# voithru/voice-activity-detection

Hardware: AMD Instinct MI355X
Metric: audio frames/sec (whole node) (higher is better)
Workload: dtype f32 (bf16x6 split operands, f32 accumulate)

## Files before the change

### __graft_entry__.py

```python
from __future__ import annotations

import sys
from pathlib import Path

REPO = Path(__file__).resolve().parent
if str(REPO) not in sys.path:
    sys.path.insert(0, str(REPO))


def build() -> None:
    from voice_activity_detection_amd import _lib, build as b

    so = b.build(force=True, verbose=True)
    b.build_variant(b.FAULT_LIB, b.FAULT_DEFINES, force=True, verbose=True)
    from oracle import oracle

    oracle.build(force=True)
    lib = _lib.load()
    import subprocess

    chk = subprocess.run([sys.executable, str(REPO / "scripts" / "check_async_loads.py"), "--lib", str(so)], capture_output=True, text=True)
    if chk.returncode != 0:
        raise RuntimeError("scripts/check_async_loads.py flags the built library:\n" + (chk.stdout + chk.stderr)[-3000:])
    import voice_activity_detection_amd as pkg

    assert pkg.SelfAttentiveVAD is not None
    print(f"built {so} [{lib.savad_version().decode()}] and {oracle.build()}")


def smoke() -> None:
    import numpy as np
    import torch

    from oracle import oracle
    from voice_activity_detection_amd import SelfAttentiveVAD, VADFromScratchPredictor, seeded_features, seeded_state_dict

    assert torch.cuda.is_available(), "smoke() needs a HIP device"
    state = seeded_state_dict(1234)
    model = SelfAttentiveVAD(80, 3, 128, 0.5)
    model.load_state_dict({k: torch.from_numpy(v) for k, v in state.items()})
    model = model.to("cuda:0").eval()
    worst = 0.0
    worst_s = 0.0
    for shape in ((8, 7, 80), (2, 96, 80)):
        x = seeded_features(7, shape)
        ref = oracle.forward(state, x)
        for prec, rm in (("fp32", 0), ("fp32s", 0)) + ((("fp32s", 7), ("fp32s", 8)) if shape[1] <= 32 else (("fp32s", 3),)):
            model.precision, model.row_mode = prec, rm
            try:
                with torch.no_grad():
                    y = model(features=torch.from_numpy(x).to("cuda:0")).cpu().numpy()
            finally:
                model.precision, model.row_mode = "fp32", 0
            err = float(np.abs(y - ref).max())
            if prec == "fp32":
                worst = max(worst, err)
            else:
                worst_s = max(worst_s, err)
            assert err < 1e-4, f"log-prob mismatch {err} at {shape} ({prec}, row_mode {rm})"
    feat = seeded_features(8, (120, 80))
    probs = VADFromScratchPredictor(model, "cuda:0").predict_probabilities(feat)
    ref_probs, _ = oracle.predict_probabilities(state, feat)
    perr = float(np.abs(probs - ref_probs).max())
    assert perr < 1e-4, perr
    x7 = seeded_features(9, (40, 7, 80))
    model.precision = "bf16"
    try:
        with torch.no_grad():
            y16 = model(features=torch.from_numpy(x7).to("cuda:0")).cpu().numpy()
    finally:
        model.precision = "fp32"
    e16 = float(np.abs(y16 - oracle.forward(state, x7)).max())
    assert e16 < 1.2e-2, f"bf16 log-prob mismatch {e16}"
    from oracle import logmel
    from voice_activity_detection_amd.features import log_mel

    audio = (np.random.default_rng(3).standard_normal(16000) * 0.1).astype(np.float32)
    emel = float(np.abs(log_mel(audio, "cuda:0").cpu().numpy() - logmel.log_mel(audio)).max())
    assert emel < 5e-4, f"log-mel mismatch {emel}"
    from oracle import resample as oresample
    from voice_activity_detection_amd.features import resample_to_16k_device

    clip = (np.random.default_rng(4).standard_normal(4000) * 0.1).astype(np.float32)
    assert np.array_equal(resample_to_16k_device(torch.from_numpy(clip).to("cuda:0"), 44100).cpu().numpy(), oresample.resample(clip, 44100)), "resampler bits"
    print(f"smoke ok: max |dlogp| = {worst:.2e} (fp32s: {worst_s:.2e}), predictor max |dp| = {perr:.2e}, bf16 T=7 max |dlogp| = {e16:.2e}, log-mel max |d| = {emel:.2e}")


if __name__ == "__main__":
    build()
    if "--smoke" in sys.argv:
        smoke()
```

### voice_activity_detection_amd/build.py

```python
from __future__ import annotations

import os
import shutil
import subprocess
import sys
from pathlib import Path

PKG = Path(__file__).resolve().parent
SRC = PKG / "csrc" / "savad.hip"
DEPS = (sorted((PKG / "csrc").glob("*.h")) + sorted((PKG / "csrc").glob("*.hip")) + sorted((PKG / "csrc").glob("*.inc")) +
        [PKG.parent / "include" / "savad.h"])
LIB = PKG / "libsavad.so"


def hipcc() -> str:
    for cand in (os.environ.get("HIPCC"), shutil.which("hipcc"), "/opt/rocm/bin/hipcc"):
        if cand and Path(cand).exists():
            return cand
    raise RuntimeError("hipcc not found (set HIPCC or install ROCm under /opt/rocm)")


def is_stale() -> bool:
    return not LIB.exists() or any(d.stat().st_mtime > LIB.stat().st_mtime for d in DEPS)


def build(force: bool = False, verbose: bool = False) -> Path:
    if not force and not is_stale():
        return LIB
    cmd = [hipcc(), "--offload-arch=gfx950", "-O3", "-std=c++17", "-shared", "-fPIC", "-fvisibility=hidden",
           "-Wno-unused-value", str(SRC), "-o", str(LIB)]
    if verbose:
        print(" ".join(cmd), file=sys.stderr)
    subprocess.run(cmd, check=True)
    return LIB


def build_variant(out: Path, defines=(), force: bool = False, verbose: bool = False) -> Path:
    out = Path(out)
    if not force and out.exists() and all(d.stat().st_mtime <= out.stat().st_mtime for d in DEPS):
        return out
    out.parent.mkdir(parents=True, exist_ok=True)
    cmd = [hipcc(), "--offload-arch=gfx950", "-O3", "-std=c++17", "-shared", "-fPIC", "-fvisibility=hidden", "-Wno-unused-value",
           *[f"-D{d}" for d in defines], str(SRC), "-o", str(out)]
    if verbose:
        print(" ".join(cmd), file=sys.stderr)
    subprocess.run(cmd, check=True)
    return out


FAULT_LIB = PKG.parent / "tests" / "fault" / "libsavad_fault17.so"
FAULT_DEFINES = ["SAVAD_FAULT_INJECT=17"]


if __name__ == "__main__":
    print(build(force="--force" in sys.argv, verbose=True))
```

### voice_activity_detection_amd/csrc/savad_device.h

```cpp
#pragma once
#include <hip/hip_runtime.h>
#include <stdint.h>

#include "savad_dims.h"

namespace savad {

constexpr int XLD = D + 4;
constexpr float LN_EPS = 1e-5f;
constexpr float NEG_BIG = -1.0e30f;
constexpr float RESCALE_LOG2 = 16.0f;

typedef float f32x2 __attribute__((ext_vector_type(2)));
typedef float f32x4 __attribute__((ext_vector_type(4)));
typedef float f32x16 __attribute__((ext_vector_type(16)));

#define SAVAD_MFMA(a, b, c) __builtin_amdgcn_mfma_f32_32x32x2f32((a), (b), (c), 0, 0, 0)

__device__ __forceinline__ f32x4 ld4(const float* p) { return *reinterpret_cast<const f32x4*>(p); }
__device__ __forceinline__ void st4(float* p, f32x4 v) { *reinterpret_cast<f32x4*>(p) = v; }
__device__ __forceinline__ void both_halves(float v, float& lo, float& hi) {
    const unsigned u = __builtin_bit_cast(unsigned, v);
    const auto r = __builtin_amdgcn_permlane32_swap(u, u, false, false);
    const unsigned a = r[0], b = r[1];
    lo = __builtin_bit_cast(float, a);
    hi = __builtin_bit_cast(float, b);
}
__device__ __forceinline__ float half_sum(float v) {
    float lo, hi;
    both_halves(v, lo, hi);
    return lo + hi;
}
__device__ __forceinline__ float half_max(float v) {
    float lo, hi;
    both_halves(v, lo, hi);
    return fmaxf(lo, hi);
}

__device__ __forceinline__ f32x16 zero16() {
    f32x16 z;
#pragma unroll
    for (int i = 0; i < 16; ++i) z[i] = 0.0f;
    return z;
}

__device__ __forceinline__ void add_bias(f32x16& acc, const float* __restrict__ b, int h) {
#pragma unroll
    for (int g = 0; g < 4; ++g) {
        const f32x4 b4 = ld4(b + 8 * g + 4 * h);
#pragma unroll
        for (int s = 0; s < 4; ++s) acc[4 * g + s] += b4[s];
    }
}

__device__ __forceinline__ size_t x_row_offset(size_t r, int T, int F, long xbs) {
    return xbs == (long)T * F ? r * (size_t)F : (r / (size_t)T) * (size_t)xbs + (r % (size_t)T) * (size_t)F;
}

__device__ __forceinline__ void store_block(float* rowp , const f32x16& v, int h) {
#pragma unroll
    for (int g = 0; g < 4; ++g) {
        f32x4 t;
#pragma unroll
        for (int s = 0; s < 4; ++s) t[s] = v[4 * g + s];
        st4(rowp + 8 * g + 4 * h, t);
    }
}
__device__ __forceinline__ void add_block(f32x16& v, const float* rowp, int h) {
#pragma unroll
    for (int g = 0; g < 4; ++g) {
        const f32x4 t = ld4(rowp + 8 * g + 4 * h);
#pragma unroll
        for (int s = 0; s < 4; ++s) v[4 * g + s] += t[s];
    }
}

__device__ __forceinline__ void layernorm_regs(const f32x16 (&x)[4], f32x4 (&xg)[16]) {
    float s = 0.0f;
#pragma unroll
    for (int nb = 0; nb < 4; ++nb)
#pragma unroll
        for (int r = 0; r < 16; ++r) s += x[nb][r];
    s = half_sum(s);
    const float mean = s * (1.0f / D);
    float ss = 0.0f;
#pragma unroll
    for (int nb = 0; nb < 4; ++nb)
#pragma unroll
        for (int r = 0; r < 16; ++r) {
            const float d = x[nb][r] - mean;
            xg[4 * nb + (r >> 2)][r & 3] = d;
            ss += d * d;
        }
    ss = half_sum(ss);
    const float rstd = 1.0f / sqrtf(ss * (1.0f / D) + LN_EPS);
#pragma unroll
    for (int G = 0; G < 16; ++G) xg[G] *= rstd;
}

__device__ __forceinline__ void wait_vmem_all() {
    __builtin_amdgcn_s_waitcnt(0x0F70);
    asm volatile("" ::: "memory");
}

__device__ __forceinline__ bool xcd_balanced_map(int B, int per_seq, int& b, int& rr) {
    const long W = (long)B * per_seq;
    const int per_xcd = (int)((W + 7) / 8);
    const int xcd = blockIdx.x & 7, slot = blockIdx.x >> 3;
    const long lin = (long)xcd * per_xcd + slot;
    if (slot >= per_xcd || lin >= W) return false;
    b = (int)(lin / per_seq);
    rr = (int)(lin % per_seq);
    return true;
}

#ifdef SAVAD_TIMING
__device__ long long g_savad_dbg[64];
#define SAVAD_STAMP(i)                                                                  \
    do {                                                                                \
        if (blockIdx.x == 0 && threadIdx.x == 0) g_savad_dbg[i] = __builtin_readcyclecounter(); \
    } while (0)
#else
#define SAVAD_STAMP(i) \
    do {               \
    } while (0)
#endif
#ifndef SAVAD_FAULT_INJECT
#define SAVAD_FAULT_INJECT 0
#endif
#ifndef SAVAD_ABLATE
#define SAVAD_ABLATE 0
#endif

__device__ __forceinline__ void stage_bias(float* dst, const float* __restrict__ src, int count) {
    for (int i = threadIdx.x * 4; i < count; i += 256 * 4) st4(dst + i, ld4(src + i));
}
struct BiasPiece {
    float* dst;
    const float* src;
    int count;
};
template <int N>
struct BiasRegs {
    f32x4 v[N];
};
template <int N>
__device__ __forceinline__ BiasRegs<N> request_bias_pieces(const BiasPiece (&p)[N]) {
    const int i = threadIdx.x * 4;
    BiasRegs<N> r;
#pragma unroll
    for (int n = 0; n < N; ++n) {
        const int j = i < p[n].count ? i : (p[n].count >= 4 ? p[n].count - 4 : 0);
        r.v[n] = ld4(p[n].src + j);
    }
    return r;
}
template <int N>
__device__ __forceinline__ void commit_bias_pieces(const BiasPiece (&p)[N], const BiasRegs<N>& r) {
    const int i = threadIdx.x * 4;
#pragma unroll
    for (int n = 0; n < N; ++n)
        if (i < p[n].count) st4(p[n].dst + i, r.v[n]);
}
template <int N>
__device__ __forceinline__ void stage_bias_pieces(const BiasPiece (&p)[N]) {
    commit_bias_pieces(p, request_bias_pieces(p));
}
__device__ __forceinline__ f32x16 bias_block(const float* lds_bias , int h) {
    f32x16 r;
#pragma unroll
    for (int g = 0; g < 4; ++g) {
        const f32x4 b4 = ld4(lds_bias + 8 * g + 4 * h);
#pragma unroll
        for (int e = 0; e < 4; ++e) r[4 * g + e] = b4[e];
    }
    return r;
}

struct WindowOffsets {
    int w;
    int off[64];
};


__device__ __forceinline__ constexpr int acc_row(int r, int h) { return 8 * (r >> 2) + 4 * h + (r & 3); }

__device__ __forceinline__ bool packed_key_ok(int B, int T, int blk, int m, int jk) {
    const int G = 32 / T;
    return (jk < G * T) && (jk / T == m / T) && (blk * G + jk / T < B);
}

__device__ __forceinline__ f32x2 classify_rows(const f32x4 (&xg)[16], const float* wc, const float* bc, int h) {
    float z0 = 0.0f, z1 = 0.0f;
#pragma unroll
    for (int G = 0; G < 16; ++G) {
        const f32x4 c0 = ld4(wc + 8 * G + 4 * h), c1 = ld4(wc + D + 8 * G + 4 * h);
#pragma unroll
        for (int e = 0; e < 4; ++e) {
            z0 = __builtin_fmaf(xg[G][e], c0[e], z0);
            z1 = __builtin_fmaf(xg[G][e], c1[e], z1);
        }
    }
    z0 = half_sum(z0) + bc[0];
    z1 = half_sum(z1) + bc[1];
    const float mx = fmaxf(z0, z1);
    const float lse = mx + logf(expf(z0 - mx) + expf(z1 - mx));
    return f32x2{z0 - lse, z1 - lse};
}

}
```

### voice_activity_detection_amd/csrc/savad_kernels_f32s.h

```cpp
#pragma once
#include "savad_kernels_bf16.h"
#include <type_traits>

namespace savad {
#ifdef SAVAD_TIMING
__device__ long long g_savad_wg[1024][4];
#endif
namespace fs {

using bf::bf16x8;
using bf::u32x4;
using bf::ldfrag;
using bf::stfrag;
using bf::FRAG_BYTES;
using bf::slot_row;
using bf::AttnState;
using bf::attn_state_init;
using bf::online_softmax_shifted;

constexpr int SLOT_BYTES = 2 * BLK3_BYTES;
constexpr int NRING3 = 3;
constexpr int ROW_LDS_BYTES = NRING3 * SLOT_BYTES + 9 * D * 4;

struct Tri {
    bf16x8 h, m, l;
};

__device__ __forceinline__ void split1(float a, __bf16& h, __bf16& m, __bf16& l) {
    h = (__bf16)a;
    if (SAVAD_ABLATE & 128) {
        m = l = h;
        return;
    }
    const float r1 = a - (float)h;
    m = (__bf16)r1;
    const float r2 = r1 - (float)m;
    l = (__bf16)r2;
}
__device__ __forceinline__ Tri split8(const float (&v)[8]) {
    Tri t;
#pragma unroll
    for (int e = 0; e < 8; ++e) {
        __bf16 h, m, l;
        split1(v[e], h, m, l);
        t.h[e] = h;
        t.m[e] = m;
        t.l[e] = l;
    }
    return t;
}
__device__ __forceinline__ Tri split_half(const f32x16& v, int j) {
    float t[8];
#pragma unroll
    for (int e = 0; e < 8; ++e) t[e] = v[8 * j + e];
    return split8(t);
}
__device__ __forceinline__ void split_row(const f32x4 (&xg)[16], Tri (&xp)[8]) {
#pragma unroll
    for (int ks = 0; ks < 8; ++ks) {
        float t[8];
#pragma unroll
        for (int e = 0; e < 8; ++e) t[e] = xg[2 * ks + (e >> 2)][e & 3];
        xp[ks] = split8(t);
    }
}
__device__ __forceinline__ Tri ldtri(const char* p ) {
    return Tri{ldfrag(p), ldfrag(p + FRAG_BYTES), ldfrag(p + 2 * FRAG_BYTES)};
}
__device__ __forceinline__ void sttri(char* p, const Tri& t) {
    stfrag(p, t.h);
    stfrag(p + FRAG_BYTES, t.m);
    stfrag(p + 2 * FRAG_BYTES, t.l);
}
__device__ __forceinline__ Tri zero_tri() {
    const bf16x8 z = __builtin_bit_cast(bf16x8, u32x4{0u, 0u, 0u, 0u});
    return Tri{z, z, z};
}

#define SAVAD_MF(a, b, c) __builtin_amdgcn_mfma_f32_32x32x16_bf16((a), (b), (c), 0, 0, 0)
template <bool SWAP>
__device__ __forceinline__ void mfma6x2_lo(f32x16& acc0, f32x16& acc1, const Tri& a0, const Tri& a1, const Tri& b) {
#define SAVAD_MF2(pa, pb)                                                           \
    acc0 = SWAP ? SAVAD_MF(b.pb, a0.pa, acc0) : SAVAD_MF(a0.pa, b.pb, acc0);        \
    acc1 = SWAP ? SAVAD_MF(b.pb, a1.pa, acc1) : SAVAD_MF(a1.pa, b.pb, acc1);
    SAVAD_MF2(h, l) SAVAD_MF2(l, h) SAVAD_MF2(m, m)
}
template <bool SWAP>
__device__ __forceinline__ void mfma6x2_hi(f32x16& acc0, f32x16& acc1, const Tri& a0, const Tri& a1, const Tri& b) {
    SAVAD_MF2(h, m) SAVAD_MF2(m, h) SAVAD_MF2(h, h)
#undef SAVAD_MF2
}
template <bool SWAP>
__device__ __forceinline__ void mfma6x2(f32x16& acc0, f32x16& acc1, const Tri& a0, const Tri& a1, const Tri& b) {
    mfma6x2_lo<SWAP>(acc0, acc1, a0, a1, b);
    mfma6x2_hi<SWAP>(acc0, acc1, a0, a1, b);
}

__device__ __forceinline__ void load_hblock32(f32x16 (&x)[4], const float* hb, int lane) {
#pragma unroll
    for (int nb = 0; nb < 4; ++nb)
#pragma unroll
        for (int g = 0; g < 4; ++g) {
            const f32x4 t = ld4(hb + ((nb * 4 + g) * 64 + lane) * 4);
#pragma unroll
            for (int s = 0; s < 4; ++s) x[nb][4 * g + s] += t[s];
        }
}
__device__ __forceinline__ void request_hblock32(f32x4 (&hr)[16], const float* hb , int lane) {
#define SAVAD_H_LD(i)                                                                                                          \
    asm volatile("global_load_dwordx4 %0, %1, %2 offset:%3" : "+v"(hr[i]) : "v"((unsigned)lane * 16u + 4096u * ((i) / 4)), "s"(hb), \
                 "n"(((i) % 4) * 1024) : "memory")
    SAVAD_H_LD(0); SAVAD_H_LD(1); SAVAD_H_LD(2); SAVAD_H_LD(3); SAVAD_H_LD(4); SAVAD_H_LD(5); SAVAD_H_LD(6); SAVAD_H_LD(7);
    SAVAD_H_LD(8); SAVAD_H_LD(9); SAVAD_H_LD(10); SAVAD_H_LD(11); SAVAD_H_LD(12); SAVAD_H_LD(13); SAVAD_H_LD(14); SAVAD_H_LD(15);
#undef SAVAD_H_LD
}
__device__ __forceinline__ void landed_hblock32(f32x4 (&hr)[16]) {
    asm volatile("" : "+v"(hr[0]), "+v"(hr[1]), "+v"(hr[2]), "+v"(hr[3]), "+v"(hr[4]), "+v"(hr[5]), "+v"(hr[6]), "+v"(hr[7]), "+v"(hr[8]),
                 "+v"(hr[9]), "+v"(hr[10]), "+v"(hr[11]), "+v"(hr[12]), "+v"(hr[13]), "+v"(hr[14]), "+v"(hr[15]));
}
__device__ __forceinline__ void store_hblock32(float* hb, const f32x16 (&x)[4], int lane) {
#pragma unroll
    for (int nb = 0; nb < 4; ++nb)
#pragma unroll
        for (int g = 0; g < 4; ++g) {
            f32x4 t;
#pragma unroll
            for (int s = 0; s < 4; ++s) t[s] = x[nb][4 * g + s];
            st4(hb + ((nb * 4 + g) * 64 + lane) * 4, t);
        }
}

#ifndef SAVAD_PIECE_FENCE
#define SAVAD_PIECE_FENCE 0x6
#endif
__device__ __forceinline__ const char* scalar_ptr(const char* p) {
    const size_t a = (size_t)p;
    const unsigned lo = __builtin_amdgcn_readfirstlane((unsigned)a), hi = __builtin_amdgcn_readfirstlane((unsigned)(a >> 32));
    return (const char*)((size_t)lo | ((size_t)hi << 32));
}
struct DmaJob {
    const char* src;
    unsigned ldsb;
};
struct Ring3 {
    static constexpr int PER = 12;
    char* base;
    int w, lane;
    unsigned voff[3];

    __device__ __forceinline__ Ring3(char* smem, int w_, int lane_) : base(smem), w(w_), lane(lane_) {
#pragma unroll
        for (int g = 0; g < 3; ++g) voff[g] = (unsigned)lane_ * 16u + 4096u * g;
    }
    __device__ __forceinline__ char* slot(int t) const { return base + (t % NRING3) * SLOT_BYTES; }
    __device__ __forceinline__ DmaJob job(int t, const char* seg0, const char* seg1) const {
        const unsigned slot0 = __builtin_amdgcn_readfirstlane((unsigned)(size_t)slot(t));
        return DmaJob{((w >> 1) ? seg1 : seg0) + (size_t)(w & 1) * (BLK3_BYTES / 2), slot0 + (unsigned)w * (BLK3_BYTES / 2)};
    }
    template <int I>
    __device__ __forceinline__ void piece(const DmaJob& j) const {
        if (SAVAD_ABLATE & 1) return;
        __builtin_amdgcn_sched_barrier(SAVAD_PIECE_FENCE);
        piece_raw<I>(j);
        __builtin_amdgcn_sched_barrier(SAVAD_PIECE_FENCE);
    }
    template <int I>
    __device__ __forceinline__ void piece_raw(const DmaJob& j) const {
        asm volatile(
            "s_add_u32 m0, %2, %3\n\t"
            "s_nop 0\n\t"
            "global_load_lds_dwordx4 %0, %1 offset:%4"
            :
            : "v"(voff[I / 4]), "s"(j.src), "s"(j.ldsb), "n"((I / 4) * 4096), "n"((I % 4) * 1024)
            : "memory", "scc");
    }
    __device__ __forceinline__ void issue_all(const DmaJob& j) const {
        if (SAVAD_ABLATE & 1) return;
        piece_raw<0>(j); piece_raw<1>(j); piece_raw<2>(j); piece_raw<3>(j); piece_raw<4>(j); piece_raw<5>(j);
        piece_raw<6>(j); piece_raw<7>(j); piece_raw<8>(j); piece_raw<9>(j); piece_raw<10>(j); piece_raw<11>(j);
    }
    template <int NEWER>
    __device__ __forceinline__ void acquire() const {
        if (SAVAD_ABLATE & 2) return;
        __builtin_amdgcn_s_waitcnt(bf::Ring<4>::vmcnt_imm(NEWER * PER));
        asm volatile("" ::: "memory");
        __syncthreads();
    }
};

struct NoMid {
    template <int KS>
    __device__ __forceinline__ void operator()(std::integral_constant<int, KS>) const {}
};
template <bool SWAP, bool DMA, class Mid = NoMid>
__device__ __forceinline__ void gemm_slot(f32x16& acc0, f32x16& acc1, const char* slot, const Tri (&xp)[8], const Ring3& ring,
                                          const DmaJob& job, const Mid& mid = Mid{}) {
    if (SAVAD_ABLATE & 8) {
#pragma unroll
        for (int ks = 0; ks < 8; ++ks) mfma6x2<SWAP>(acc0, acc1, xp[7 - ks], xp[ks ^ 1], xp[ks]);
        return;
    }
    const unsigned a = (unsigned)(size_t)slot + (unsigned)ring.lane * 16u;
    u32x4 f[2][6];
#define SAVAD_G_LD(ks, i) asm volatile("ds_read_b128 %0, %1 offset:%2" : "=v"(f[(ks) & 1][i]) : "v"(a), "n"(((i) / 3) * BLK3_BYTES + (ks) * TFRAG_BYTES + ((i) % 3) * FRAG_BYTES))
#define SAVAD_G_LD6(ks) SAVAD_G_LD(ks, 0); SAVAD_G_LD(ks, 1); SAVAD_G_LD(ks, 2); SAVAD_G_LD(ks, 3); SAVAD_G_LD(ks, 4); SAVAD_G_LD(ks, 5)
#define SAVAD_G_STEP(ks, P0, P1)                                                                                              \
    {                                                                                                                         \
        if constexpr ((ks) + 1 < 8) { SAVAD_G_LD6((ks) + 1); }                                                                \
        asm volatile("s_waitcnt lgkmcnt(%6)"                                                                                  \
                     : "+v"(f[(ks) & 1][0]), "+v"(f[(ks) & 1][1]), "+v"(f[(ks) & 1][2]), "+v"(f[(ks) & 1][3]), "+v"(f[(ks) & 1][4]), \
                       "+v"(f[(ks) & 1][5])                                                                                   \
                     : "n"((ks) + 1 < 8 ? 6 : 0));                                                                            \
        const Tri w0_{__builtin_bit_cast(bf16x8, f[(ks) & 1][0]), __builtin_bit_cast(bf16x8, f[(ks) & 1][1]),                  \
                      __builtin_bit_cast(bf16x8, f[(ks) & 1][2])};                                                            \
        const Tri w1_{__builtin_bit_cast(bf16x8, f[(ks) & 1][3]), __builtin_bit_cast(bf16x8, f[(ks) & 1][4]),                  \
                      __builtin_bit_cast(bf16x8, f[(ks) & 1][5])};                                                            \
        mfma6x2_lo<SWAP>(acc0, acc1, w0_, w1_, xp[ks]);                                                                       \
        if constexpr (DMA && (P1) >= 0) ring.template piece<((P1) >= 0 ? (P1) : 0)>(job);                                     \
        mid(std::integral_constant<int, (ks)>{});                                                                             \
        mfma6x2_hi<SWAP>(acc0, acc1, w0_, w1_, xp[ks]);                                                                       \
        if constexpr (DMA) ring.template piece<P0>(job);                                                                      \
    }
    SAVAD_G_LD6(0);
    SAVAD_G_STEP(0, 1, 0) SAVAD_G_STEP(1, 2, -1) SAVAD_G_STEP(2, 4, 3) SAVAD_G_STEP(3, 5, -1)
    SAVAD_G_STEP(4, 7, 6) SAVAD_G_STEP(5, 8, -1) SAVAD_G_STEP(6, 10, 9) SAVAD_G_STEP(7, 11, -1)
#undef SAVAD_G_STEP
#undef SAVAD_G_LD6
#undef SAVAD_G_LD
}

__global__ void pack_weight_frags3_kernel(const float* __restrict__ W, int N, int K, __bf16* __restrict__ out) {
    const int KS = K / 16;
    const size_t total = (size_t)(N / 32) * KS * 64 * 8;
    for (size_t i = (size_t)blockIdx.x * blockDim.x + threadIdx.x; i < total; i += (size_t)gridDim.x * blockDim.x) {
        const int e = (int)(i & 7);
        const int lane = (int)((i >> 3) & 63);
        const size_t f = i >> 9;
        const int ks = (int)(f % KS);
        const int nblk = (int)(f / KS);
        const int n = lane & 31, h = lane >> 5;
        const int k = 32 * (ks >> 1) + 16 * (ks & 1) + 8 * (e >> 2) + 4 * h + (e & 3);
        __bf16 ph, pm, pl;
        split1(W[(size_t)(32 * nblk + n) * K + k], ph, pm, pl);
        const size_t o = f * 3 * 512 + (size_t)lane * 8 + e;
        out[o] = ph;
        out[o + 512] = pm;
        out[o + 1024] = pl;
    }
}

__global__ void fold_vo_kernel(const float* __restrict__ Wo, const float* __restrict__ Wv, const float* __restrict__ bqkv,
                               float* __restrict__ Wvo, float* __restrict__ bvo) {
    const int n = blockIdx.x, k = threadIdx.x;
    double acc = 0.0, accb = 0.0;
    for (int j = 0; j < D; ++j) {
        const double w = (double)Wo[(size_t)n * D + j];
        acc += w * (double)Wv[(size_t)j * D + k];
        accb += w * (double)bqkv[2 * D + j];
    }
    Wvo[(size_t)n * D + k] = (float)acc;
    if (k == 0) bvo[n] = (float)accb;
}

__global__ void fold_qk_kernel(const float* __restrict__ Wq, const float* __restrict__ Wk, const float* __restrict__ bq, double c,
                               float* __restrict__ Wqt, float* __restrict__ bqt) {
    const int n = blockIdx.x, k = threadIdx.x;
    double acc = 0.0, accb = 0.0;
    for (int o = 0; o < D; ++o) {
        const double w = (double)Wk[(size_t)o * D + n];
        acc += w * (double)Wq[(size_t)o * D + k];
        accb += w * (double)bq[o];
    }
    Wqt[(size_t)n * D + k] = (float)(c * acc);
    if (k == 0) bqt[n] = (float)(c * accb);
}

template <int RB, int HALF, bool DMA, bool SCALE, class Mid = NoMid>
__device__ __forceinline__ void qkv_slot(const char* slot, const Tri (&xp)[8], const float* lb, char* __restrict__ dst, int blk,
                                         const Ring3& ring, const DmaJob& job, float qscale, bool live, const Mid& mid = Mid{}) {
    const int lane = ring.lane, n = lane & 31, h = lane >> 5;
    constexpr int nb0 = 2 * HALF;
    f32x16 acc[2];
    if constexpr (RB < 2) {
#pragma unroll
        for (int i = 0; i < 2; ++i) acc[i] = bias_block(lb + 32 * (nb0 + i), h);
        gemm_slot<false, DMA>(acc[0], acc[1], slot, xp, ring, job, mid);
    } else {
#pragma unroll
        for (int i = 0; i < 2; ++i) {
            const float bv = lb[32 * (nb0 + i) + n];
#pragma unroll
            for (int r = 0; r < 16; ++r) acc[i][r] = bv;
        }
        gemm_slot<true, DMA>(acc[0], acc[1], slot, xp, ring, job, mid);
    }
    if constexpr (SCALE) {
        acc[0] *= qscale;
        acc[1] *= qscale;
    }
    if (!live) return;
#pragma unroll
    for (int i = 0; i < 2; ++i)
#pragma unroll
        for (int j = 0; j < 2; ++j)
            sttri(dst + (size_t)blk * BLK3_BYTES + (2 * (nb0 + i) + j) * TFRAG_BYTES + lane * 16, split_half(acc[i], j));
}
template <int S, bool QKF, bool DMA, class Mid = NoMid>
__device__ __forceinline__ void qkv_image_slot(const char* slot, const Tri (&xp)[8], const float* lbq, char* __restrict__ qf, char* __restrict__ kf,
                                               char* __restrict__ vtf, int blk, const Ring3& ring, const DmaJob& job, float qscale, bool live,
                                               const Mid& mid = Mid{}) {
    constexpr int pos = S >> 1, rb = QKF ? 2 * pos : pos;
    qkv_slot<rb, (S & 1), DMA, (rb == 0 && !QKF)>(slot, xp, lbq + D * pos, rb == 0 ? qf : (rb == 1 ? kf : vtf), blk, ring, job, qscale, live, mid);
}

#ifndef SAVAD_KSTORE
#define SAVAD_KSTORE 2
#endif
__device__ __forceinline__ void store_k_tri(char* kblk , const Tri (&xp)[8], int ks, int lane) {
    sttri(kblk + ks * TFRAG_BYTES + lane * 16, xp[ks]);
}
__device__ __forceinline__ void store_k_burst(char* kblk, const Tri (&xp)[8], int lane, bool live) {
    if (!live) return;
#pragma unroll
    for (int ks = 0; ks < 8; ++ks) store_k_tri(kblk, xp, ks, lane);
}
template <int S>
struct KStoreMid {
    char* kblk;
    const Tri (&xp)[8];
    int lane;
    bool live;
    template <int KS>
    __device__ __forceinline__ void operator()(std::integral_constant<int, KS>) const {
        if constexpr ((KS & 1) && ((SAVAD_KSTORE == 2 && S == 0) || SAVAD_KSTORE == 3)) {
            __builtin_amdgcn_sched_barrier(SAVAD_PIECE_FENCE);
            if (live) {
                if constexpr (SAVAD_KSTORE == 2) {
                    store_k_tri(kblk, xp, KS - 1, lane);
                    store_k_tri(kblk, xp, KS, lane);
                } else {
                    store_k_tri(kblk, xp, 4 * S + (KS >> 1), lane);
                }
            }
            __builtin_amdgcn_sched_barrier(SAVAD_PIECE_FENCE);
        }
    }
};

__device__ __forceinline__ Tri load_x_tri(const float* p, bool valid) {
    f32x4 a = __builtin_nontemporal_load(reinterpret_cast<const f32x4*>(p)), b = __builtin_nontemporal_load(reinterpret_cast<const f32x4*>(p + 8));
    if (!valid) a = b = f32x4{0.f, 0.f, 0.f, 0.f};
    float t[8];
#pragma unroll
    for (int e = 0; e < 4; ++e) {
        t[e] = a[e];
        t[4 + e] = b[e];
    }
    return split8(t);
}

__device__ __forceinline__ void input_gemm_f32s(f32x16 (&h0)[4], const float* xr, bool valid, const char* win, int KS, int lane, int h) {
    constexpr int KSMAX = 8;
    f32x4 xa[KSMAX], xc[KSMAX];
#pragma unroll
    for (int ks = 0; ks < KSMAX; ++ks) {
        const int kc = ks < KS ? ks : KS - 1;
        const float* px = xr + 32 * (kc >> 1) + 16 * (kc & 1) + 4 * h;
        xa[ks] = __builtin_nontemporal_load(reinterpret_cast<const f32x4*>(px));
        xc[ks] = __builtin_nontemporal_load(reinterpret_cast<const f32x4*>(px + 8));
    }
    auto wtri = [&](int nb, int ks) { return ldtri(win + (size_t)(nb * KS + (ks < KS ? ks : KS - 1)) * TFRAG_BYTES + lane * 16); };
    Tri wn[4] = {wtri(0, 0), wtri(1, 0), wtri(2, 0), wtri(3, 0)};
#pragma unroll
    for (int ks = 0; ks < KSMAX; ++ks)
        if (ks < KS) {
            const Tri w0 = wn[0], w1 = wn[1], w2 = wn[2], w3 = wn[3];
            if (ks + 1 < KSMAX) {
#pragma unroll
                for (int nb = 0; nb < 4; ++nb) wn[nb] = wtri(nb, ks + 1);
            }
            float t[8];
#pragma unroll
            for (int e = 0; e < 4; ++e) {
                t[e] = valid ? xa[ks][e] : 0.0f;
                t[4 + e] = valid ? xc[ks][e] : 0.0f;
            }
            const Tri xf = split8(t);
            mfma6x2<false>(h0[0], h0[1], w0, w1, xf);
            mfma6x2<false>(h0[2], h0[3], w2, w3, xf);
        }
    for (int ks = KSMAX; ks < KS; ++ks) {
        const int f0 = 32 * (ks >> 1) + 16 * (ks & 1) + 4 * h;
        const Tri xf = load_x_tri(xr + f0, valid);
#pragma unroll
        for (int nb = 0; nb < 4; nb += 2)
            mfma6x2<false>(h0[nb], h0[nb + 1], ldtri(win + (size_t)(nb * KS + ks) * TFRAG_BYTES + lane * 16),
                           ldtri(win + (size_t)((nb + 1) * KS + ks) * TFRAG_BYTES + lane * 16), xf);
    }
}

template <bool QKF>
__device__ __forceinline__ void input_qkv_f32s(char* smem, const float* __restrict__ x, long xbs, int B, int T, int F, int nblk,
                                               const char* __restrict__ win_frag, const float* __restrict__ bin, const float* __restrict__ pe,
                                               const char* __restrict__ wqkv_frag, const float* __restrict__ bqkv, float* __restrict__ hbuf,
                                               char* __restrict__ qf, char* __restrict__ kf, char* __restrict__ vtf, float qscale) {
    float* lbq = reinterpret_cast<float*>(smem + NRING3 * SLOT_BYTES);
    const int lane = threadIdx.x & 63, m = lane & 31, h = lane >> 5;
    const int w = __builtin_amdgcn_readfirstlane(threadIdx.x >> 6);
    const int blk = blockIdx.x * 4 + w;
    const Ring3 ring(smem, w, lane);
    auto job = [&](int t) { return ring.job(t, wqkv_frag + (size_t)(2 * t) * BLK3_BYTES, wqkv_frag + (size_t)(2 * t + 1) * BLK3_BYTES); };
    SAVAD_STAMP(57);
    ring.issue_all(job(0));
    ring.issue_all(job(1));
    stage_bias(lbq, bqkv, (QKF ? 2 : 3) * D);
    SAVAD_STAMP(58);
    size_t row;
    int t_frame;
    const bool valid = (blk < nblk) && slot_row(B, T, blk, m, row, t_frame);
    if (!valid) {
        row = 0;
        t_frame = 0;
    }
    f32x16 h0[4];
#pragma unroll
    for (int nb = 0; nb < 4; ++nb) {
        h0[nb] = zero16();
        add_bias(h0[nb], bin + 32 * nb, h);
        add_block(h0[nb], pe + (size_t)t_frame * D + 32 * nb, h);
    }
    input_gemm_f32s(h0, x + x_row_offset(row, T, F, xbs), valid, win_frag, F / 16, lane, h);
    SAVAD_STAMP(59);
    const bool live = blk < nblk;
    if (live) store_hblock32(hbuf + (size_t)blk * (32 * D), h0, lane);
    f32x4 xg[16];
    layernorm_regs(h0, xg);
    Tri xp[8];
    split_row(xg, xp);
    SAVAD_STAMP(60);
    const DmaJob none{nullptr, 0u};
    constexpr int NS = QKF ? 4 : 6;
    char* kblk = kf + (size_t)blk * BLK3_BYTES;
#define SAVAD_IQ_STEP(T_, mid)                                                                                                 \
    ring.acquire<((T_) + 1 < NS) ? 1 : 0>();                                                                                   \
    if (QKF && SAVAD_KSTORE == 1 && (T_) == 0) store_k_burst(kblk, xp, lane, live);                                            \
    qkv_image_slot<T_, QKF, ((T_) + 2 < NS)>(ring.slot(T_), xp, lbq, qf, kf, vtf, blk, ring, (T_) + 2 < NS ? job((T_) + 2) : none, qscale, \
                                             live, mid);
    if constexpr (QKF) {
        if (SAVAD_KSTORE == 0) store_k_burst(kblk, xp, lane, live);
        SAVAD_IQ_STEP(0, (KStoreMid<0>{kblk, xp, lane, live})) SAVAD_IQ_STEP(1, (KStoreMid<1>{kblk, xp, lane, live}))
        SAVAD_STAMP(61);
        SAVAD_IQ_STEP(2, NoMid{}) SAVAD_IQ_STEP(3, NoMid{})
        SAVAD_STAMP(63);
    } else {
        SAVAD_IQ_STEP(0, NoMid{}) SAVAD_IQ_STEP(1, NoMid{})
        SAVAD_STAMP(61);
        SAVAD_IQ_STEP(2, NoMid{}) SAVAD_IQ_STEP(3, NoMid{})
        SAVAD_STAMP(62);
        SAVAD_IQ_STEP(4, NoMid{}) SAVAD_IQ_STEP(5, NoMid{})
        SAVAD_STAMP(63);
    }
#undef SAVAD_IQ_STEP
}
__global__ __launch_bounds__(256, 1) void input_qkv_kernel_f32s(const float* __restrict__ x, long xbs, int B, int T, int F, int nblk,
                                                                const char* __restrict__ win_frag, const float* __restrict__ bin,
                                                                const float* __restrict__ pe, const char* __restrict__ wqkv_frag,
                                                                const float* __restrict__ bqkv, float* __restrict__ hbuf,
                                                                char* __restrict__ qf, char* __restrict__ kf, char* __restrict__ vtf,
                                                                float qscale) {
    extern __shared__ __attribute__((aligned(16))) char smem[];
    input_qkv_f32s<true>(smem, x, xbs, B, T, F, nblk, win_frag, bin, pe, wqkv_frag, bqkv, hbuf, qf, kf, vtf, qscale);
}
__global__ __launch_bounds__(256, 1) void input_qkv_kernel_f32s_plain(const float* __restrict__ x, long xbs, int B, int T, int F, int nblk,
                                                                      const char* __restrict__ win_frag, const float* __restrict__ bin,
                                                                      const float* __restrict__ pe, const char* __restrict__ wqkv_frag,
                                                                      const float* __restrict__ bqkv, float* __restrict__ hbuf,
                                                                      char* __restrict__ qf, char* __restrict__ kf, char* __restrict__ vtf,
                                                                      float qscale) {
    extern __shared__ __attribute__((aligned(16))) char smem[];
    input_qkv_f32s<false>(smem, x, xbs, B, T, F, nblk, win_frag, bin, pe, wqkv_frag, bqkv, hbuf, qf, kf, vtf, qscale);
}

typedef __bf16 bf16x2 __attribute__((ext_vector_type(2)));
__device__ __forceinline__ void split_pair(float a0, float a1, unsigned& h, unsigned& m, unsigned& l) {
    __bf16 h0, m0, l0, h1, m1, l1;
    split1(a0, h0, m0, l0);
    split1(a1, h1, m1, l1);
    h = __builtin_bit_cast(unsigned, bf16x2{h0, h1});
    m = __builtin_bit_cast(unsigned, bf16x2{m0, m1});
    l = __builtin_bit_cast(unsigned, bf16x2{l0, l1});
}
__device__ __forceinline__ void settle_reference(f32x16& sc, AttnState& st, bool first ) {
    float mx = sc[0];
#pragma unroll
    for (int r = 1; r < 16; ++r) mx = fmaxf(mx, sc[r]);
    mx = half_max(mx);
    const bool move = (mx > RESCALE_LOG2) || (first && mx < -RESCALE_LOG2);
    if (__any(move)) {
        const float d = move ? mx : 0.0f;
        if (!first) {
            const float alpha = __builtin_amdgcn_exp2f(-d);
            st.l_run *= alpha;
#pragma unroll
            for (int nb = 0; nb < 4; ++nb) st.O[nb] *= alpha;
        }
#pragma unroll
        for (int r = 0; r < 16; ++r) {
            sc[r] -= d;
            st.negm[r] -= d;
        }
    }
}
__device__ __forceinline__ f32x16 qk_tile3(const AttnState& st, const Tri (&qp)[8], const char* kblk, int lane) {
    f32x16 sa = st.negm, sb = zero16();
#pragma unroll
    for (int ks = 0; ks < 8; ++ks) {
        const Tri k = ldtri(kblk + ks * TFRAG_BYTES + lane * 16);
        sa = SAVAD_MF(k.h, qp[ks].l, sa);
        sb = SAVAD_MF(k.l, qp[ks].h, sb);
        sa = SAVAD_MF(k.m, qp[ks].m, sa);
        sb = SAVAD_MF(k.h, qp[ks].m, sb);
        sa = SAVAD_MF(k.m, qp[ks].h, sa);
        sb = SAVAD_MF(k.h, qp[ks].h, sb);
    }
    return sa + sb;
}
template <bool HAVE_NEXT, bool DMA, class MaskNext>
__device__ __forceinline__ void attn_step3(AttnState& st, const Tri (&qp)[8], f32x16& sc, const char* slot, MaskNext mask_next,
                                           const Ring3& ring, const DmaJob& job) {
    const unsigned av = (unsigned)(size_t)slot + (unsigned)ring.lane * 16u, ak = av + BLK3_BYTES;
    f32x16 sa = st.negm, sb = zero16();
    unsigned ph[8], pm[8], pl[8];
    float rs = 0.0f;
    u32x4 fk[3][3];
    u32x4 fv[2][6];
#define SAVAD_A_LDK(ks, i) asm volatile("ds_read_b128 %0, %1 offset:%2" : "=v"(fk[(ks) % 3][i]) : "v"(ak), "n"((ks) * TFRAG_BYTES + (i) * FRAG_BYTES))
#define SAVAD_A_LDK3(ks) SAVAD_A_LDK(ks, 0); SAVAD_A_LDK(ks, 1); SAVAD_A_LDK(ks, 2)
#define SAVAD_A_LDV(g, i) asm volatile("ds_read_b128 %0, %1 offset:%2" : "=v"(fv[(g) & 1][i]) : "v"(av), "n"((((2 * ((g) >> 1) + (i) / 3) * 2 + ((g) & 1)) * 3 + (i) % 3) * FRAG_BYTES))
#define SAVAD_A_LDV6(g) SAVAD_A_LDV(g, 0); SAVAD_A_LDV(g, 1); SAVAD_A_LDV(g, 2); SAVAD_A_LDV(g, 3); SAVAD_A_LDV(g, 4); SAVAD_A_LDV(g, 5)
#define SAVAD_A_SOFT(ks)                                                                                                       \
    {                                                                                                                          \
        const float e0_ = (SAVAD_ABLATE & 4) ? sc[2 * (ks)] : __builtin_amdgcn_exp2f(sc[2 * (ks)]);                            \
        const float e1_ = (SAVAD_ABLATE & 4) ? sc[2 * (ks) + 1] : __builtin_amdgcn_exp2f(sc[2 * (ks) + 1]);                    \
        rs += e0_;                                                                                                             \
        rs += e1_;                                                                                                             \
        split_pair(e0_, e1_, ph[ks], pm[ks], pl[ks]);                                                                          \
    }
#define SAVAD_A_QK(ks)                                                                                                         \
    {                                                                                                                          \
        if constexpr ((ks) + 2 < 8) { SAVAD_A_LDK3((ks) + 2); }                                                                \
        if constexpr ((ks) == 6) { SAVAD_A_LDV6(0); }                                                                          \
        asm volatile("s_waitcnt lgkmcnt(%3)" : "+v"(fk[(ks) % 3][0]), "+v"(fk[(ks) % 3][1]), "+v"(fk[(ks) % 3][2])             \
                     : "n"((ks) + 2 < 8 ? 6 : ((ks) == 6 ? 9 : 6)));                                                           \
        const bf16x8 kh_ = __builtin_bit_cast(bf16x8, fk[(ks) % 3][0]), km_ = __builtin_bit_cast(bf16x8, fk[(ks) % 3][1]),     \
                     kl_ = __builtin_bit_cast(bf16x8, fk[(ks) % 3][2]);                                                        \
        sa = SAVAD_MF(kh_, qp[ks].l, sa);                                                                                      \
        sb = SAVAD_MF(kl_, qp[ks].h, sb);                                                                                      \
        sa = SAVAD_MF(km_, qp[ks].m, sa);                                                                                      \
        sb = SAVAD_MF(kh_, qp[ks].m, sb);                                                                                      \
        sa = SAVAD_MF(km_, qp[ks].h, sa);                                                                                      \
        sb = SAVAD_MF(kh_, qp[ks].h, sb);                                                                                      \
        SAVAD_A_SOFT(ks)                                                                                                       \
    }
    if constexpr (HAVE_NEXT) {
        SAVAD_A_LDK3(0);
        SAVAD_A_LDK3(1);
        SAVAD_A_QK(0) SAVAD_A_QK(1) SAVAD_A_QK(2) SAVAD_A_QK(3) SAVAD_A_QK(4) SAVAD_A_QK(5) SAVAD_A_QK(6) SAVAD_A_QK(7)
    } else {
        SAVAD_A_LDV6(0);
        SAVAD_A_SOFT(0) SAVAD_A_SOFT(1) SAVAD_A_SOFT(2) SAVAD_A_SOFT(3) SAVAD_A_SOFT(4) SAVAD_A_SOFT(5) SAVAD_A_SOFT(6) SAVAD_A_SOFT(7)
    }
#undef SAVAD_A_QK
#undef SAVAD_A_SOFT
#undef SAVAD_A_LDK3
#undef SAVAD_A_LDK
    st.l_run += rs;
    const Tri p0{__builtin_bit_cast(bf16x8, u32x4{ph[0], ph[1], ph[2], ph[3]}), __builtin_bit_cast(bf16x8, u32x4{pm[0], pm[1], pm[2], pm[3]}),
                 __builtin_bit_cast(bf16x8, u32x4{pl[0], pl[1], pl[2], pl[3]})};
    const Tri p1{__builtin_bit_cast(bf16x8, u32x4{ph[4], ph[5], ph[6], ph[7]}), __builtin_bit_cast(bf16x8, u32x4{pm[4], pm[5], pm[6], pm[7]}),
                 __builtin_bit_cast(bf16x8, u32x4{pl[4], pl[5], pl[6], pl[7]})};
#define SAVAD_A_PV(g, PJ)                                                                                                      \
    {                                                                                                                          \
        if constexpr ((g) + 1 < 4) { SAVAD_A_LDV6((g) + 1); }                                                                  \
        asm volatile("s_waitcnt lgkmcnt(%6)"                                                                                   \
                     : "+v"(fv[(g) & 1][0]), "+v"(fv[(g) & 1][1]), "+v"(fv[(g) & 1][2]), "+v"(fv[(g) & 1][3]), "+v"(fv[(g) & 1][4]), \
                       "+v"(fv[(g) & 1][5])                                                                                    \
                     : "n"((g) + 1 < 4 ? 6 : 0));                                                                              \
        const Tri v0_{__builtin_bit_cast(bf16x8, fv[(g) & 1][0]), __builtin_bit_cast(bf16x8, fv[(g) & 1][1]),                   \
                      __builtin_bit_cast(bf16x8, fv[(g) & 1][2])};                                                             \
        const Tri v1_{__builtin_bit_cast(bf16x8, fv[(g) & 1][3]), __builtin_bit_cast(bf16x8, fv[(g) & 1][4]),                   \
                      __builtin_bit_cast(bf16x8, fv[(g) & 1][5])};                                                             \
        mfma6x2<false>(st.O[2 * ((g) >> 1)], st.O[2 * ((g) >> 1) + 1], v0_, v1_, PJ);                                          \
        if constexpr (DMA) {                                                                                                   \
            ring.template piece<3 * (g)>(job);                                                                                 \
            ring.template piece<3 * (g) + 1>(job);                                                                             \
            ring.template piece<3 * (g) + 2>(job);                                                                             \
        }                                                                                                                      \
    }
    SAVAD_A_PV(0, p0) SAVAD_A_PV(1, p1)
    if constexpr (HAVE_NEXT) {
        sc = sa + sb;
        mask_next(sc);
    }
    SAVAD_A_PV(2, p0) SAVAD_A_PV(3, p1)
#undef SAVAD_A_PV
#undef SAVAD_A_LDV6
#undef SAVAD_A_LDV
    if constexpr (HAVE_NEXT) settle_reference(sc, st, false);
}
template <class Mask>
__device__ __forceinline__ void attn_tile3_global(AttnState& st, const Tri (&qp)[8], const char* kblk, const char* vtblk, Mask mask, int lane) {
    f32x16 sa = st.negm, sb = zero16();
#pragma unroll
    for (int ks = 0; ks < 8; ++ks) {
        const Tri k = ldtri(kblk + ks * TFRAG_BYTES + lane * 16);
        sa = SAVAD_MF(k.h, qp[ks].l, sa);
        sb = SAVAD_MF(k.l, qp[ks].h, sb);
        sa = SAVAD_MF(k.m, qp[ks].m, sa);
        sb = SAVAD_MF(k.h, qp[ks].m, sb);
        sa = SAVAD_MF(k.m, qp[ks].h, sa);
        sb = SAVAD_MF(k.h, qp[ks].h, sb);
    }
    f32x16 sc = sa + sb;
    mask(sc);
    online_softmax_shifted(sc, st, true);
    const Tri p0 = split_half(sc, 0), p1 = split_half(sc, 1);
#pragma unroll
    for (int nbd = 0; nbd < 4; nbd += 2) {
        mfma6x2<false>(st.O[nbd], st.O[nbd + 1], ldtri(vtblk + ((nbd * 2 + 0) * TFRAG_BYTES) + lane * 16),
                       ldtri(vtblk + (((nbd + 1) * 2 + 0) * TFRAG_BYTES) + lane * 16), p0);
        mfma6x2<false>(st.O[nbd], st.O[nbd + 1], ldtri(vtblk + ((nbd * 2 + 1) * TFRAG_BYTES) + lane * 16),
                       ldtri(vtblk + (((nbd + 1) * 2 + 1) * TFRAG_BYTES) + lane * 16), p1);
    }
}

struct RowArgs3 {
    int B, T, nblk;
    float* hbuf;
    const char* wo_frag;
    const float* bo;
    const char* w1_frag;
    const float* b1;
    const char* w2_frag;
    const float* b2;
    const char* wn_frag;
    const float* wc;
    const float* bn;
    char *qf, *kf, *vtf;
    float* out;
    float qscale;
};
__device__ __forceinline__ const char* row_seg(const RowArgs3& A, int t, int sgm, bool folded) {
    if (!folded) {
        if (t < 2) return A.wo_frag + (size_t)(2 * t + sgm) * BLK3_BYTES;
        t -= 2;
    }
    if (t < 16) {
        const int c = t >> 2, r = t & 3;
        return r < 2 ? A.w1_frag + (size_t)(4 * c + 2 * r + sgm) * BLK3_BYTES
                     : A.w2_frag + (size_t)((2 * (r - 2) + sgm) * 32 + 8 * c) * TFRAG_BYTES;
    }
    return A.wn_frag + (size_t)(2 * (t - 16) + sgm) * BLK3_BYTES;
}

__host__ __device__ constexpr int row_slots(bool last, bool folded) { return (folded ? 0 : 2) + (last ? 16 : folded ? 20 : 22); }

template <bool LAST, bool FOLDED>
struct RowBiases {
    BiasPiece pieces[4];
    BiasRegs<4> regs;
    float bc;
    float* lbn;
    __device__ __forceinline__ RowBiases(const RowArgs3& A, char* smem) {
        float* lbo = reinterpret_cast<float*>(smem + NRING3 * SLOT_BYTES);
        float* lb1 = lbo + D;
        float* lb2 = lb1 + DFF;
        lbn = lb2 + D;
        pieces[0] = BiasPiece{lbo, A.bo, D};
        pieces[1] = BiasPiece{lb1, A.b1, DFF};
        pieces[2] = BiasPiece{lb2, A.b2, D};
        pieces[3] = BiasPiece{lbn, LAST ? A.wc : A.bn, (LAST || FOLDED) ? 2 * D : 3 * D};
        regs = request_bias_pieces(pieces);
        bc = LAST ? A.bn[threadIdx.x & 1] : 0.0f;
    }
    __device__ __forceinline__ void commit() const {
        commit_bias_pieces(pieces, regs);
        if (LAST && threadIdx.x < 2) lbn[2 * D + threadIdx.x] = bc;
    }
};

template <bool LAST, bool FOLDED>
__device__ __forceinline__ void row_stage_f32s(const RowArgs3& A, char* smem, Tri (&xp)[8], const f32x16 (&hc)[4], f32x4 (&hr)[16], int blk,
                                               bool live, const Ring3& ring, int base) {
    float* lbo = reinterpret_cast<float*>(smem + NRING3 * SLOT_BYTES);
    float* lb1 = lbo + D;
    float* lb2 = lb1 + DFF;
    float* lbn = lb2 + D;
    const int lane = ring.lane, m = lane & 31, h = lane >> 5;
    constexpr int OFF = FOLDED ? 0 : 2;
    constexpr int NSLOT = row_slots(LAST, FOLDED);
    auto job = [&](int t) { return ring.job(base + t, row_seg(A, t, 0, FOLDED), row_seg(A, t, 1, FOLDED)); };
    const DmaJob none{nullptr, 0u};
#define SAVAD_ROW_GEMM(T_, acc0, acc1, operand)                                                                               \
    if ((T_) < 8) SAVAD_STAMP(24 + 3 * (T_));                                                                                 \
    if constexpr (!(FOLDED && (T_) == 0)) ring.acquire<((T_) + 1 < NSLOT) ? 1 : 0>();    \
    if ((T_) < 8) SAVAD_STAMP(25 + 3 * (T_));                                                                                 \
    gemm_slot<false, ((T_) + 2 < NSLOT)>(acc0, acc1, ring.slot(base + (T_)), operand, ring, (T_) + 2 < NSLOT ? job((T_) + 2) : none); \
    if ((T_) < 8) SAVAD_STAMP(26 + 3 * (T_));
    float* hb = A.hbuf + (size_t)blk * (32 * D);
    f32x16 h1[4];
    if constexpr (FOLDED) {
        ring.acquire<1>();
        landed_hblock32(hr);
#pragma unroll
        for (int nb = 0; nb < 4; ++nb) {
            h1[nb] = bias_block(lbo + 32 * nb, h) + hc[nb];
#pragma unroll
            for (int r = 0; r < 16; ++r) h1[nb][r] += hr[4 * nb + (r >> 2)][r & 3];
        }
    } else {
        ring.issue_all(job(0));
        ring.issue_all(job(1));
        ring.acquire<1>();
        f32x16 hres[4];
#pragma unroll
        for (int nb = 0; nb < 4; ++nb) hres[nb] = zero16();
        if (live) load_hblock32(hres, hb, lane);
#pragma unroll
        for (int nb = 0; nb < 4; ++nb) h1[nb] = bias_block(lbo + 32 * nb, h);
        gemm_slot<false, true>(h1[0], h1[1], ring.slot(base), xp, ring, job(2));
        SAVAD_ROW_GEMM(1, h1[2], h1[3], xp)
#pragma unroll
        for (int nb = 0; nb < 4; ++nb) h1[nb] += hres[nb];
    }
// ... 725 lines not shown
```

Baseline: 90.06 million.

## Hand-schedule input GEMM prologue with interleaved weight-ring DMA pieces

For the QKF path with F=80, the kernel now has a hand-written prologue. It issues bias, positional-encoding, feature and input-weight loads as inline global_load asm. It double-buffers weight fragments across k-steps and spreads the 24 QKV weight-ring DMA pieces between the split-bf16 MFMA halves, instead of issuing the whole ring up front and then running the generic input GEMM. The goal is to overlap global-memory latency with MFMA work in the first stage. The cost is more live VGPRs, hard-coded vmcnt counts and a KS=5-only code path, with a legacy build variant kept for comparison.

```diff
diff --git a/__graft_entry__.py b/__graft_entry__.py
--- a/__graft_entry__.py
+++ b/__graft_entry__.py
@@ -13,6 +13,7 @@
 
     so = b.build(force=True, verbose=True)
     b.build_variant(b.FAULT_LIB, b.FAULT_DEFINES, force=True, verbose=True)
+    b.build_variant(b.LEGACY_LIB, b.LEGACY_DEFINES, force=True, verbose=True)
     from oracle import oracle
 
     oracle.build(force=True)
diff --git a/voice_activity_detection_amd/build.py b/voice_activity_detection_amd/build.py
--- a/voice_activity_detection_amd/build.py
+++ b/voice_activity_detection_amd/build.py
@@ -50,6 +50,8 @@
 
 FAULT_LIB = PKG.parent / "tests" / "fault" / "libsavad_fault17.so"
 FAULT_DEFINES = ["SAVAD_FAULT_INJECT=17"]
+LEGACY_LIB = PKG.parent / "tests" / "fault" / "libsavad_prologue_legacy.so"
+LEGACY_DEFINES = ["SAVAD_PROLOGUE_LEGACY"]
 
 
 if __name__ == "__main__":
diff --git a/voice_activity_detection_amd/csrc/savad_device.h b/voice_activity_detection_amd/csrc/savad_device.h
--- a/voice_activity_detection_amd/csrc/savad_device.h
+++ b/voice_activity_detection_amd/csrc/savad_device.h
@@ -163,6 +163,15 @@
         if (i < p[n].count) st4(p[n].dst + i, r.v[n]);
 }
 template <int N>
+__device__ __forceinline__ void request_bias_pieces_by_hand(const BiasPiece (&p)[N], BiasRegs<N>& r) {
+    const int i = threadIdx.x * 4;
+#pragma unroll
+    for (int n = 0; n < N; ++n) {
+        const int j = i < p[n].count ? i : (p[n].count >= 4 ? p[n].count - 4 : 0);
+        asm volatile("global_load_dwordx4 %0, %1, off" : "=v"(r.v[n]) : "v"(p[n].src + j) : "memory");
+    }
+}
+template <int N>
 __device__ __forceinline__ void stage_bias_pieces(const BiasPiece (&p)[N]) {
     commit_bias_pieces(p, request_bias_pieces(p));
 }
diff --git a/voice_activity_detection_amd/csrc/savad_kernels_f32s.h b/voice_activity_detection_amd/csrc/savad_kernels_f32s.h
--- a/voice_activity_detection_amd/csrc/savad_kernels_f32s.h
+++ b/voice_activity_detection_amd/csrc/savad_kernels_f32s.h
@@ -130,6 +130,9 @@
         }
 }
 
+#ifndef SAVAD_PROLOGUE_LEGACY
+#define SAVAD_PROLOGUE_LEGACY 0
+#endif
 #ifndef SAVAD_PIECE_FENCE
 #define SAVAD_PIECE_FENCE 0x6
 #endif
@@ -399,6 +402,107 @@
     }
 }
 
+template <int KS>
+__device__ __forceinline__ void input_stage_by_hand(f32x16 (&h0)[4], float* lbq, const float* bqkv, int nbias, const float* bin,
+                                                    const float* pe_row , const float* xr , bool valid,
+                                                    const char* win, const Ring3& ring, const DmaJob& j0, const DmaJob& j1, int h) {
+    static_assert(4 + 5 * (KS - 1) == 2 * Ring3::PER, "the deal of the 24 pieces is written for KS = 5");
+    wait_vmem_all();
+    const BiasPiece bp[1] = {BiasPiece{lbq, bqkv, nbias}};
+    BiasRegs<1> br;
+    request_bias_pieces_by_hand(bp, br);
+    f32x4 bi[16], pr[16], xf[2 * KS];
+    u32x4 wf[2][12];
+    const unsigned vh = (unsigned)h * 16u, vl = (unsigned)ring.lane * 16u;
+    const float *ppe = pe_row + 4 * h, *px = xr + 4 * h;
+#define SAVAD_IN_LDB(i) asm volatile("global_load_dwordx4 %0, %1, %2 offset:%3" : "=v"(bi[i]) : "v"(vh), "s"(bin), "n"(128 * ((i) / 4) + 32 * ((i) % 4)) : "memory")
+#define SAVAD_IN_LDP(i) asm volatile("global_load_dwordx4 %0, %1, off offset:%2" : "=v"(pr[i]) : "v"(ppe), "n"(128 * ((i) / 4) + 32 * ((i) % 4)) : "memory")
+#define SAVAD_IN_LDX(i) asm volatile("global_load_dwordx4 %0, %1, off offset:%2 nt" : "=v"(xf[i]) : "v"(px), "n"(32 * (i)) : "memory")
+#define SAVAD_IN_LDW(ks, i)                                                                                                    \
+    asm volatile("global_load_dwordx4 %0, %1, %2 offset:%3" : "=v"(wf[(ks) & 1][i]) : "v"(vl), "s"(win + (size_t)(((i) / 3) * KS + (ks)) * TFRAG_BYTES), \
+                 "n"(((i) % 3) * FRAG_BYTES) : "memory")
+#define SAVAD_IN_LDW12(ks)                                                                                                     \
+    SAVAD_IN_LDW(ks, 0); SAVAD_IN_LDW(ks, 1); SAVAD_IN_LDW(ks, 2); SAVAD_IN_LDW(ks, 3); SAVAD_IN_LDW(ks, 4); SAVAD_IN_LDW(ks, 5);       \
+    SAVAD_IN_LDW(ks, 6); SAVAD_IN_LDW(ks, 7); SAVAD_IN_LDW(ks, 8); SAVAD_IN_LDW(ks, 9); SAVAD_IN_LDW(ks, 10); SAVAD_IN_LDW(ks, 11)
+    SAVAD_IN_LDB(0); SAVAD_IN_LDB(1); SAVAD_IN_LDB(2); SAVAD_IN_LDB(3); SAVAD_IN_LDB(4); SAVAD_IN_LDB(5); SAVAD_IN_LDB(6); SAVAD_IN_LDB(7);
+    SAVAD_IN_LDB(8); SAVAD_IN_LDB(9); SAVAD_IN_LDB(10); SAVAD_IN_LDB(11); SAVAD_IN_LDB(12); SAVAD_IN_LDB(13); SAVAD_IN_LDB(14); SAVAD_IN_LDB(15);
+    SAVAD_IN_LDP(0); SAVAD_IN_LDP(1); SAVAD_IN_LDP(2); SAVAD_IN_LDP(3); SAVAD_IN_LDP(4); SAVAD_IN_LDP(5); SAVAD_IN_LDP(6); SAVAD_IN_LDP(7);
+    SAVAD_IN_LDP(8); SAVAD_IN_LDP(9); SAVAD_IN_LDP(10); SAVAD_IN_LDP(11); SAVAD_IN_LDP(12); SAVAD_IN_LDP(13); SAVAD_IN_LDP(14); SAVAD_IN_LDP(15);
+    SAVAD_IN_LDX(0); SAVAD_IN_LDX(1); SAVAD_IN_LDX(2); SAVAD_IN_LDX(3); SAVAD_IN_LDX(4); SAVAD_IN_LDX(5); SAVAD_IN_LDX(6); SAVAD_IN_LDX(7);
+    SAVAD_IN_LDX(8); SAVAD_IN_LDX(9);
+    static_assert(KS == 5, "ten feature pieces are requested");
+    SAVAD_IN_LDW12(0);
+    __builtin_amdgcn_s_waitcnt(bf::Ring<4>::vmcnt_imm(0));
+    asm volatile("" : "+v"(br.v[0]), "+v"(xf[0]), "+v"(xf[1]), "+v"(xf[2]), "+v"(xf[3]), "+v"(xf[4]), "+v"(xf[5]), "+v"(xf[6]), "+v"(xf[7]),
+                 "+v"(xf[8]), "+v"(xf[9]));
+    asm volatile("" : "+v"(bi[0]), "+v"(bi[1]), "+v"(bi[2]), "+v"(bi[3]), "+v"(bi[4]), "+v"(bi[5]), "+v"(bi[6]), "+v"(bi[7]), "+v"(bi[8]),
+                 "+v"(bi[9]), "+v"(bi[10]), "+v"(bi[11]), "+v"(bi[12]), "+v"(bi[13]), "+v"(bi[14]), "+v"(bi[15]));
+    asm volatile("" : "+v"(pr[0]), "+v"(pr[1]), "+v"(pr[2]), "+v"(pr[3]), "+v"(pr[4]), "+v"(pr[5]), "+v"(pr[6]), "+v"(pr[7]), "+v"(pr[8]),
+                 "+v"(pr[9]), "+v"(pr[10]), "+v"(pr[11]), "+v"(pr[12]), "+v"(pr[13]), "+v"(pr[14]), "+v"(pr[15]));
+    asm volatile("" : "+v"(wf[0][0]), "+v"(wf[0][1]), "+v"(wf[0][2]), "+v"(wf[0][3]), "+v"(wf[0][4]), "+v"(wf[0][5]), "+v"(wf[0][6]),
+                 "+v"(wf[0][7]), "+v"(wf[0][8]), "+v"(wf[0][9]), "+v"(wf[0][10]), "+v"(wf[0][11]));
+    commit_bias_pieces(bp, br);
+#pragma unroll
+    for (int nb = 0; nb < 4; ++nb) {
+        h0[nb] = zero16();
+#pragma unroll
+        for (int r = 0; r < 16; ++r) h0[nb][r] += bi[4 * nb + (r >> 2)][r & 3];
+#pragma unroll
+        for (int r = 0; r < 16; ++r) h0[nb][r] += pr[4 * nb + (r >> 2)][r & 3];
+    }
+    auto xtri = [&](int ks) {
+        float t[8];
+#pragma unroll
+        for (int e = 0; e < 4; ++e) {
+            t[e] = valid ? xf[2 * ks][e] : 0.0f;
+            t[4 + e] = valid ? xf[2 * ks + 1][e] : 0.0f;
+        }
+        return split8(t);
+    };
+    Tri xs[2];
+    xs[0] = xtri(0);
+#define SAVAD_IN_PIECE(C)                                                                                                      \
+    __builtin_amdgcn_sched_barrier(0);                                                                                         \
+    if constexpr ((C) < Ring3::PER) ring.template piece_raw<((C) < Ring3::PER ? (C) : 0)>(j0);                                 \
+    else ring.template piece_raw<((C) < Ring3::PER ? 0 : (C) - Ring3::PER)>(j1);                                               \
+    __builtin_amdgcn_sched_barrier(0);
+#define SAVAD_IN_STEP(ks, C0, NEWER)                                                                                           \
+    {                                                                                                                          \
+        if constexpr ((ks) + 1 < KS) { SAVAD_IN_LDW12((ks) + 1); }                                                             \
+        if constexpr ((ks) > 0) {                                                                                              \
+            asm volatile("s_waitcnt vmcnt(%12)"                                                                                \
+                         : "+v"(wf[(ks) & 1][0]), "+v"(wf[(ks) & 1][1]), "+v"(wf[(ks) & 1][2]), "+v"(wf[(ks) & 1][3]), "+v"(wf[(ks) & 1][4]), \
+                           "+v"(wf[(ks) & 1][5]), "+v"(wf[(ks) & 1][6]), "+v"(wf[(ks) & 1][7]), "+v"(wf[(ks) & 1][8]), "+v"(wf[(ks) & 1][9]), \
+                           "+v"(wf[(ks) & 1][10]), "+v"(wf[(ks) & 1][11])                                                      \
+                         : "n"(NEWER));                                                                                        \
+            SAVAD_IN_PIECE(C0)                                                                                                 \
+        }                                                                                                                      \
+        const Tri w0_{__builtin_bit_cast(bf16x8, wf[(ks) & 1][0]), __builtin_bit_cast(bf16x8, wf[(ks) & 1][1]), __builtin_bit_cast(bf16x8, wf[(ks) & 1][2])}; \
+        const Tri w1_{__builtin_bit_cast(bf16x8, wf[(ks) & 1][3]), __builtin_bit_cast(bf16x8, wf[(ks) & 1][4]), __builtin_bit_cast(bf16x8, wf[(ks) & 1][5])}; \
+        const Tri w2_{__builtin_bit_cast(bf16x8, wf[(ks) & 1][6]), __builtin_bit_cast(bf16x8, wf[(ks) & 1][7]), __builtin_bit_cast(bf16x8, wf[(ks) & 1][8])}; \
+        const Tri w3_{__builtin_bit_cast(bf16x8, wf[(ks) & 1][9]), __builtin_bit_cast(bf16x8, wf[(ks) & 1][10]), __builtin_bit_cast(bf16x8, wf[(ks) & 1][11])}; \
+        const Tri x_ = xs[(ks) & 1];                                                                                           \
+        constexpr int c_ = (ks) > 0 ? (C0) + 1 : (C0);                                                                         \
+        mfma6x2_lo<false>(h0[0], h0[1], w0_, w1_, x_);                                                                         \
+        if constexpr ((ks) + 1 < KS) xs[((ks) + 1) & 1] = xtri((ks) + 1);          \
+        SAVAD_IN_PIECE(c_)                                                                                                     \
+        mfma6x2_hi<false>(h0[0], h0[1], w0_, w1_, x_);                                                                         \
+        SAVAD_IN_PIECE(c_ + 1)                                                                                                 \
+        mfma6x2_lo<false>(h0[2], h0[3], w2_, w3_, x_);                                                                         \
+        SAVAD_IN_PIECE(c_ + 2)                                                                                                 \
+        mfma6x2_hi<false>(h0[2], h0[3], w2_, w3_, x_);                                                                         \
+        SAVAD_IN_PIECE(c_ + 3)                                                                                                 \
+    }
+    SAVAD_IN_STEP(0, 0, 0) SAVAD_IN_STEP(1, 4, 4 + 12) SAVAD_IN_STEP(2, 9, 5 + 12) SAVAD_IN_STEP(3, 14, 5 + 12) SAVAD_IN_STEP(4, 19, 5)
+#undef SAVAD_IN_STEP
+#undef SAVAD_IN_PIECE
+#undef SAVAD_IN_LDW12
+#undef SAVAD_IN_LDW
+#undef SAVAD_IN_LDX
+#undef SAVAD_IN_LDP
+#undef SAVAD_IN_LDB
+}
+
 template <bool QKF>
 __device__ __forceinline__ void input_qkv_f32s(char* smem, const float* __restrict__ x, long xbs, int B, int T, int F, int nblk,
                                                const char* __restrict__ win_frag, const float* __restrict__ bin, const float* __restrict__ pe,
@@ -411,9 +515,13 @@
     const Ring3 ring(smem, w, lane);
     auto job = [&](int t) { return ring.job(t, wqkv_frag + (size_t)(2 * t) * BLK3_BYTES, wqkv_frag + (size_t)(2 * t + 1) * BLK3_BYTES); };
     SAVAD_STAMP(57);
-    ring.issue_all(job(0));
-    ring.issue_all(job(1));
-    stage_bias(lbq, bqkv, (QKF ? 2 : 3) * D);
+    constexpr int KSH = 5;
+    const bool by_hand = QKF && !SAVAD_PROLOGUE_LEGACY && F == 16 * KSH;
+    if (!by_hand) {
+        ring.issue_all(job(0));
+        ring.issue_all(job(1));
+        stage_bias(lbq, bqkv, (QKF ? 2 : 3) * D);
+    }
     SAVAD_STAMP(58);
     size_t row;
     int t_frame;
@@ -423,13 +531,19 @@
         t_frame = 0;
     }
     f32x16 h0[4];
-#pragma unroll
-    for (int nb = 0; nb < 4; ++nb) {
-        h0[nb] = zero16();
-        add_bias(h0[nb], bin + 32 * nb, h);
-        add_block(h0[nb], pe + (size_t)t_frame * D + 32 * nb, h);
-    }
-    input_gemm_f32s(h0, x + x_row_offset(row, T, F, xbs), valid, win_frag, F / 16, lane, h);
+    if (by_hand) {
+        if constexpr (QKF && !SAVAD_PROLOGUE_LEGACY)
+            input_stage_by_hand<KSH>(h0, lbq, bqkv, 2 * D, bin, pe + (size_t)t_frame * D, x + x_row_offset(row, T, F, xbs), valid, win_frag, ring,
+                                     job(0), job(1), h);
+    } else {
+#pragma unroll
+        for (int nb = 0; nb < 4; ++nb) {
+            h0[nb] = zero16();
+            add_bias(h0[nb], bin + 32 * nb, h);
+            add_block(h0[nb], pe + (size_t)t_frame * D + 32 * nb, h);
+        }
+        input_gemm_f32s(h0, x + x_row_offset(row, T, F, xbs), valid, win_frag, F / 16, lane, h);
+    }
     SAVAD_STAMP(59);
     const bool live = blk < nblk;
     if (live) store_hblock32(hbuf + (size_t)blk * (32 * D), h0, lane);
```

Result: no change. 90.14 million (median of 2 runs) (+0.1%).
